# cyberfabric/cyberfabric-core

Measured on NVIDIA H100. Metric: prompt_bytes_per_sec_bpe_encode, higher is better.
Workload: dtype u32

## Files before the change

cyberfabric-core_b200/csrc/bpe_kernels.cuh:

```cuda
#pragma once
#include <stdint.h>

#include "pretok.cuh"
#include "pretok_fsm.h"
#include "pretok_sync.cuh"
#include "specials.h"
#include "tables.h"
#include "tma.cuh"

namespace cfbpe {

#ifdef CUSIM_EMULATOR
#define CFBPE_DYN_SMEM(name) uint32_t* const name = reinterpret_cast<uint32_t*>(cusim::dyn_smem())
#else
#define CFBPE_DYN_SMEM(name) extern __shared__ __align__(16) uint32_t name[]
#endif

constexpr uint32_t kMaxVocabs = 8;
#ifdef CUSIM_EMULATOR
inline unsigned long long* dbg_counters() { static unsigned long long c[16]; return c; }
#define CFBPE_DBG_COUNT(i) (++dbg_counters()[i])
#else
#define CFBPE_DBG_COUNT(i) ((void)0)
#endif
// ... 297 lines not shown
#endif
        }
    }
    if (!kFix) {
        or_bits(piece_bits, cs >> 5, static_cast<uint32_t>(mine));
        or_bits(piece_bits, (cs >> 5) + 1, static_cast<uint32_t>(mine >> 32));
    }
    if (bad) atomicOr(&status->bad_utf8, 1u);
}

__global__ void __launch_bounds__(256)
pretok_split_kernel(BatchView b, VocabSet vs, UcTables uc, uint32_t* __restrict__ piece_bits, DeviceStatus* status, SplitFix* fix_list, uint32_t fix_cap) {
    __shared__ uint16_t s_fsm[kNumPatterns * kPretokTableSize];
    __shared__ uint8_t s_ascii[128];
    for (uint32_t i = threadIdx.x; i < kNumPatterns * kPretokTableSize; i += blockDim.x) s_fsm[i] = uc.fsm[i];
    if (threadIdx.x < 128) s_ascii[threadIdx.x] = uc.ascii_x[threadIdx.x];
    __syncthreads();
    const uint64_t chunk = static_cast<uint64_t>(blockIdx.x) * blockDim.x + threadIdx.x;
    const uint64_t cs = chunk * kSplitChunk;
    if (cs >= b.total_bytes) return;
    const uint64_t ce = (cs + kSplitChunk < b.total_bytes) ? cs + kSplitChunk : b.total_bytes;
    split_thread<0>(b, vs, uc, s_fsm, s_ascii, piece_bits, status, fix_list, fix_cap, cs, ce, 0, 0);
}

__global__ void __launch_bounds__(256)
pretok_fixup_kernel(BatchView b, VocabSet vs, UcTables uc, uint32_t* __restrict__ piece_bits, DeviceStatus* status, const SplitFix* fix_list, uint32_t fix_cap) {
    __shared__ uint16_t s_fsm[kNumPatterns * kPretokTableSize];
    __shared__ uint8_t s_ascii[128];
    const uint32_t n = status->fix_n < fix_cap ? status->fix_n : fix_cap;
    if (blockIdx.x * blockDim.x >= n) return;
    for (uint32_t i = threadIdx.x; i < kNumPatterns * kPretokTableSize; i += blockDim.x) s_fsm[i] = uc.fsm[i];
    if (threadIdx.x < 128) s_ascii[threadIdx.x] = uc.ascii_x[threadIdx.x];
    __syncthreads();
    for (uint32_t i = blockIdx.x * blockDim.x + threadIdx.x; i < n; i += gridDim.x * blockDim.x) {
        const SplitFix f = fix_list[i];
        split_thread<1>(b, vs, uc, s_fsm, s_ascii, piece_bits, status, nullptr, 0, 0, f.ce, f.pos, 0xFFFFFFFFu);
    }
}


constexpr uint32_t kFull = 0xFFFFFFFFu;

__device__ __forceinline__ uint32_t lanemask_lt(uint32_t lane) { return (1u << lane) - 1u; }

__device__ __forceinline__ uint64_t load_bits33(const uint32_t* __restrict__ bits, uint64_t n_words, uint64_t ws) {
    const uint64_t w = ws >> 5;
    const uint32_t sh = static_cast<uint32_t>(ws & 31);
    const uint64_t lo = bits[w];
    const uint64_t hi = (w + 1 < n_words) ? bits[w + 1] : 0;
    const uint64_t v = (lo | (hi << 32)) >> sh;
    return v & 0x1FFFFFFFFull;
}

__device__ __forceinline__ uint64_t next_set_bit(const uint32_t* __restrict__ bits, uint64_t from, uint64_t limit) {
    if (from >= limit) return limit;
    uint64_t w = from >> 5;
    uint32_t cur = bits[w] & (kFull << (from & 31));
    const uint64_t wl = (limit + 31) >> 5;
    while (!cur) {
        if (++w >= wl) return limit;
        cur = bits[w];
    }
    const uint64_t p = (w << 5) + (__ffs(cur) - 1);
    return p < limit ? p : limit;
}


constexpr uint32_t kPieceRange = 512;
constexpr uint32_t kPieceWarps = 4;

__device__ __forceinline__ void load16(const uint8_t* __restrict__ p, uint32_t& w0, uint32_t& w1, uint32_t& w2, uint32_t& w3) {
    const uintptr_t addr = reinterpret_cast<uintptr_t>(p);
    const uint32_t* q = reinterpret_cast<const uint32_t*>(addr & ~static_cast<uintptr_t>(3));
    const uint32_t sh = static_cast<uint32_t>(addr & 3) * 8;
    const uint32_t a = q[0], bq = q[1], c = q[2], d = q[3];
    if (sh == 0) { w0 = a; w1 = bq; w2 = c; w3 = d; }
    else {
        const uint32_t e = q[4];
        w0 = __funnelshift_r(a, bq, sh); w1 = __funnelshift_r(bq, c, sh); w2 = __funnelshift_r(c, d, sh); w3 = __funnelshift_r(d, e, sh);
    }
}

__device__ __forceinline__ uint32_t whole_piece_lookup(const TablesView& T, const uint8_t* __restrict__ p, uint32_t len) {
    if (len > T.max_token_len) return kNone;
    uint32_t w0, w1, w2, w3;
    load16(p, w0, w1, w2, w3);
    uint64_t k0 = static_cast<uint64_t>(w0) | (static_cast<uint64_t>(w1) << 32);
    uint32_t k1 = w2;
    if (len < 8) k0 &= (1ull << (8 * len)) - 1ull;
    if (len <= 8) k1 = 0; else if (len < 12) k1 &= (1u << (8 * (len - 8))) - 1u;
    if (len <= kShortMaxLen) return short_lookup(T, k0, k1, len);
    return long_lookup(T, long_hash(k0, k1, load_le32(p + len - 4), len), p, len);
}

__device__ __forceinline__ uint32_t merge_piece_in_lane(const TablesView& T, const uint8_t* __restrict__ text, uint64_t pos, uint32_t len,
                                                        uint32_t* sid, uint32_t* srk, uint32_t* __restrict__ tok_bits) {
    const uint8_t* __restrict__ p = text + pos;
    uint32_t w[8];
    load16(p, w[0], w[1], w[2], w[3]);
    if (len > 16) load16(p + 16, w[4], w[5], w[6], w[7]); else { w[4] = w[5] = w[6] = w[7] = 0; }
    auto byte_at = [&](uint32_t k) -> uint32_t {
        const uint32_t lo4 = (k & 4u) ? ((k & 8u) ? ((k & 16u) ? w[7] : w[3]) : ((k & 16u) ? w[5] : w[1]))
                                       : ((k & 8u) ? ((k & 16u) ? w[6] : w[2]) : ((k & 16u) ? w[4] : w[0]));
        return (lo4 >> (8u * (k & 3u))) & 0xFFu;
    };
    for (uint32_t k0 = 0; k0 < len; k0 += 4) {
        uint32_t bv[5], idv[4], rkv[4];
#pragma unroll
        for (uint32_t t = 0; t < 5; ++t) bv[t] = (k0 + t < len) ? byte_at(k0 + t) : 0u;
#pragma unroll
        for (uint32_t t = 0; t < 4; ++t) {
            idv[t] = (k0 + t < len) ? T.byte2id[bv[t]] : 0u;
            rkv[t] = (k0 + t + 1 < len) ? T.bytepair[(bv[t] << 8) | bv[t + 1]] : kNone;
        }
#pragma unroll
        for (uint32_t t = 0; t < 4; ++t) if (k0 + t < len) { sid[(k0 + t) * 32] = idv[t]; srk[(k0 + t) * 32] = rkv[t] == kNone ? kNone : ((rkv[t] << 5) | (k0 + t)); }
    }
    uint32_t alive = (len >= 32) ? kFull : ((1u << len) - 1u);
    for (;;) {
        uint32_t bkey = kNone;
        for (uint32_t bits = alive; bits; bits &= bits - 1) {
            const uint32_t k = static_cast<uint32_t>(__ffs(bits)) - 1u;
            const uint32_t r = srk[k * 32];
            bkey = r < bkey ? r : bkey;
        }
        if (bkey == kNone) break;
        const uint32_t best = bkey >> 5, bi = bkey & 31u;
        const uint32_t above = alive & ~((2u << bi) - 1u);
        const uint32_t nb = static_cast<uint32_t>(__ffs(above)) - 1u;
        alive &= ~(1u << nb);
        sid[bi * 32] = best;
        const uint32_t above2 = alive & ~((2u << bi) - 1u);
        const uint32_t below = alive & ((1u << bi) - 1u);
        const bool wr = above2 != 0, wl = below != 0;
        const uint32_t nn = wr ? static_cast<uint32_t>(__ffs(above2)) - 1u : 0u;
        const uint32_t pv = wl ? 31u - static_cast<uint32_t>(__clz(below)) : 0u;
        uint32_t nr, nl;
        pair_lookup2(T, best, wr ? sid[nn * 32] : 0u, wr, wl ? sid[pv * 32] : 0u, best, wl, nr, nl);
        srk[bi * 32] = nr == kNone ? kNone : ((nr << 5) | bi);
        if (wl) srk[pv * 32] = nl == kNone ? kNone : ((nl << 5) | pv);
    }
    const uint64_t mask = static_cast<uint64_t>(alive) << (pos & 31);
    atomicOr(&tok_bits[pos >> 5], static_cast<uint32_t>(mask));
    if (mask >> 32) atomicOr(&tok_bits[(pos >> 5) + 1], static_cast<uint32_t>(mask >> 32));
    return alive;
}

__device__ __forceinline__ uint32_t kth_set_bit(uint32_t mask, uint32_t k) {
    for (uint32_t i = 0; i < k; ++i) mask &= mask - 1;
    return __ffs(mask) - 1;
}

constexpr uint32_t kPieceMulti = 0x80000000u;
constexpr uint32_t kPieceLong = 0xFFFFFFFEu;
constexpr uint32_t kPieceTileBytes = kPieceWarps * kPieceRange;
static_assert(kPieceTileBytes == 64 * 32, "K3 derives a word's piece tile as word >> 6");
struct DenseIds {
    uint32_t* by_piece;
    uint32_t* extras;
    uint32_t extras_cap;
    uint32_t* tile_pieces;
    uint64_t* piece_base;
};

__global__ void __launch_bounds__(kPieceWarps * 32)
long_scan_kernel(BatchView b, const uint32_t* __restrict__ piece_bits, LongPiece* __restrict__ long_list, uint32_t long_cap,
                 DeviceStatus* status, uint32_t* __restrict__ tile_pieces) {
    const uint32_t lane = threadIdx.x & 31, wic = threadIdx.x >> 5;
    const uint64_t warp = static_cast<uint64_t>(blockIdx.x) * kPieceWarps + wic;
    const uint64_t r0 = warp * kPieceRange;
    const uint64_t r1 = (r0 + kPieceRange < b.total_bytes) ? r0 + kPieceRange : b.total_bytes;
    const bool multi = b.vocab_ids != nullptr;
    const uint64_t base = r0 + 16ull * lane;
    const uint32_t my = (base < b.total_bytes) ? ((piece_bits[base >> 5] >> (16u * (lane & 1u))) & 0xFFFFu) : 0u;
    uint32_t v = my ? (16u * lane + static_cast<uint32_t>(__ffs(my)) - 1u) : 0xFFFFu;
#pragma unroll
    for (uint32_t d = 1; d < 32; d <<= 1) { const uint32_t o = __shfl_down_sync(kFull, v, d); if (lane + d < 32 && o < v) v = o; }
    uint32_t nf_rel = __shfl_down_sync(kFull, v, 1);
    if (lane == 31) nf_rel = 0xFFFFu;
    const bool any_open = __any_sync(kFull, my != 0 && nf_rel == 0xFFFFu);
    uint64_t beyond = b.total_bytes;
    if (any_open) beyond = next_set_bit(piece_bits, r1, b.total_bytes);
    const uint64_t nf = (nf_rel == 0xFFFFu) ? beyond : r0 + nf_rel;
    __shared__ uint32_t s_n[2], s_at[2], s_pieces;
    __shared__ unsigned long long s_bytes;
    if (threadIdx.x < 2) s_n[threadIdx.x] = 0;
    if (threadIdx.x == 0) { s_bytes = 0; s_pieces = 0; }
    __syncthreads();
    const uint32_t np = __reduce_add_sync(kFull, static_cast<uint32_t>(__popc(my)));
    if (lane == 0 && np) atomicAdd(&s_pieces, np);
    bool is_long = false, big = false;
    uint32_t k = 0, pv = 0;
    uint64_t pos = 0;
    if (my && r0 < b.total_bytes) {
        pos = base + (31u - static_cast<uint32_t>(__clz(my)));
        if (nf - pos > 32) {
            is_long = true;
            big = (nf - pos) > kBigPiece;
            pv = multi ? b.vocab_ids[find_prompt(b.offsets, b.n_prompts, pos)] : 0u;
            k = atomicAdd(&s_n[big ? 1 : 0], 1u);
            atomicAdd(&s_bytes, static_cast<unsigned long long>(nf - pos));
        }
    }
    __syncthreads();
    if (threadIdx.x < 2 && s_n[threadIdx.x]) s_at[threadIdx.x] = atomicAdd(threadIdx.x ? &status->n_big : &status->n_long, s_n[threadIdx.x]);
    if (threadIdx.x == 2 && s_bytes) atomicAdd(&status->long_bytes, s_bytes);
    if (threadIdx.x == 3) tile_pieces[blockIdx.x] = s_pieces;
    __syncthreads();
    if (is_long) {
        const uint32_t idx = s_at[big ? 1 : 0] + k;
        if (idx < long_cap) { LongPiece lp; lp.start = pos; lp.end = nf; lp.vocab = pv; lp.pad = 0; long_list[big ? long_cap - 1 - idx : idx] = lp; }
        else atomicOr(&status->long_overflow, 1u);
    }
}

constexpr uint32_t kLookupWarps = 4;
static_assert(kLookupWarps == kPieceWarps, "K2a's CTA is the 2 KiB tile K2s counted");
__global__ void __launch_bounds__(kLookupWarps * 32)
bpe_lookup_kernel(BatchView b, VocabSet vs, const uint32_t* __restrict__ piece_bits, DenseIds dn, MissLists ml, DeviceStatus* status) {
    __shared__ uint16_t s_pos[kLookupWarps][kPieceRange + 2];
    __shared__ uint64_t s_miss0[kLookupWarps * kPieceRange / 13 + 8];
    __shared__ uint64_t s_miss1[kLookupWarps * kPieceRange / 7 + 8];
    __shared__ uint64_t s_miss2[kLookupWarps * kPieceRange / 2 + 8];
    __shared__ uint32_t s_cnt[3], s_base[3], s_nw[kLookupWarps];
    const uint32_t lane = threadIdx.x & 31, wic = threadIdx.x >> 5;
    if (threadIdx.x < 3) s_cnt[threadIdx.x] = 0;
    const uint64_t warp = static_cast<uint64_t>(blockIdx.x) * kLookupWarps + wic;
    const uint64_t r0 = warp * kPieceRange;
    const uint8_t* __restrict__ text = b.bytes;
    const bool multi = b.vocab_ids != nullptr;
    const bool in_range = r0 < b.total_bytes;
    const uint64_t r1 = (r0 + kPieceRange < b.total_bytes) ? r0 + kPieceRange : b.total_bytes;
    uint32_t n_w = 0;
    if (in_range) {
        const uint64_t base = r0 + 16ull * lane;
// ... 1165 lines not shown
```

cyberfabric-core_b200/csrc/pipeline.cuh:

```cuda
#pragma once
#include "../../include/cfbpe.h"
#include "bpe_kernels.cuh"

namespace cfbpe {

struct Workspace {
    uint32_t* piece_bits;
    uint32_t* tok_bits;
    uint32_t* ids_by_pos;
    LongScratch lscratch;
    LongPiece* long_list;
    uint32_t long_cap;
    uint32_t* tile_counts;
    uint64_t* tile_base;
    DeviceStatus* status;
    MissLists miss;
    SplitFix* fix_list;
    uint32_t fix_cap;
    DenseIds dense;
    uint32_t* pstart_bits;
    uint32_t* block_prompt;
};

enum WsKind : uint32_t {
// ... 81 lines not shown
}

inline const char* chunk_args_error(uint32_t chunk_tokens, uint32_t overlap_tokens, const uint32_t* spans, const uint64_t* chunk_offsets) {
    if (chunk_tokens == 0) return "chunk_tokens must be at least 1";
    if (overlap_tokens >= chunk_tokens) return "overlap_tokens must be less than chunk_tokens";
    if (!spans || !chunk_offsets) return "out_spans and out_chunk_offsets are required";
    return nullptr;
}

#ifndef CFBPE_LONG_CTAS
#define CFBPE_LONG_CTAS 8
#endif
constexpr uint32_t kLongCtasPerSm = CFBPE_LONG_CTAS;
#ifndef CFBPE_LIST_CTAS
#define CFBPE_LIST_CTAS 3
#endif
constexpr uint32_t kListCtasPerSm = CFBPE_LIST_CTAS;

enum KernelIdx { K_SPLIT = 0, K_ENCODE = 1, K_LONG = 2, K_COUNT = 3, K_SCAN = 4, K_EMIT = 5, K_LIST = 6, K_LONGSCAN = 7, K_MERGE = 8 };

inline uint64_t n_flag_words(uint64_t total_bytes) { return (total_bytes + 31) >> 5; }
inline uint32_t n_scan_tiles(uint64_t total_bytes) {
    return static_cast<uint32_t>((n_flag_words(total_bytes) + kScanTileWords - 1) / kScanTileWords);
}

template <typename Stream, typename Prof>
inline void enqueue_split(const BatchView& b, const VocabSet& vs, const UcTables& uc, const Workspace& w, Stream stream, Prof* prof,
                          uint32_t sm_count) {
    const uint64_t nw = n_flag_words(b.total_bytes);
    CFBPE_ZERO(w.status, sizeof(DeviceStatus), stream);
    if (!b.total_bytes) return;
    CFBPE_ZERO(w.piece_bits, (nw + 2) * sizeof(uint32_t), stream);
    CFBPE_ZERO(w.tok_bits, (nw + 2) * sizeof(uint32_t), stream);
    CFBPE_MARK(prof, K_SPLIT, stream, true);
#ifdef CFBPE_SPLIT_LEGACY
    const uint64_t n_chunks = (b.total_bytes + kSplitChunk - 1) / kSplitChunk;
    CFBPE_LAUNCH(pretok_split_kernel, static_cast<unsigned>((n_chunks + 255) / 256), 256, stream, b, vs, uc, w.piece_bits, w.status, w.fix_list, w.fix_cap);
#else
    CFBPE_ZERO(w.pstart_bits, (nw + 2) * sizeof(uint32_t), stream);
    CFBPE_LAUNCH(prompt_map_kernel, static_cast<unsigned>((static_cast<uint64_t>(b.n_prompts) + 1 + 255) / 256), 256, stream, b, vs, w.pstart_bits, w.block_prompt, w.status);
    {
        const uint64_t n_blocks16 = (b.total_bytes + 15) / 16;
        const uint32_t n_tiles = static_cast<uint32_t>((n_blocks16 + kSplitWarpOwned - 1) / kSplitWarpOwned);
        const uint32_t n_tabs = b.vocab_ids ? kNumPatterns : 1u;
        const uint32_t cap = sm_count * CFBPE_SPLIT_CTAS;
        const uint32_t n_ctas = (n_tiles + kSplitCta / 32 - 1) / (kSplitCta / 32);
        CFBPE_LAUNCH_SMEM(pretok_split16_kernel, n_ctas < cap ? n_ctas : cap, kSplitCta, n_tabs * kProdTableBytes, stream,
                          b, vs, uc, w.pstart_bits, w.block_prompt, w.piece_bits, w.status, w.fix_list, w.fix_cap, n_tabs, n_tiles);
    }
#endif
    CFBPE_LAUNCH(pretok_fixup_kernel, 2 * sm_count, 256, stream, b, vs, uc, w.piece_bits, w.status, w.fix_list, w.fix_cap);
    CFBPE_MARK(prof, K_SPLIT, stream, false);
    const uint64_t n_warps = (b.total_bytes + kPieceRange - 1) / kPieceRange;
    CFBPE_MARK(prof, K_LONGSCAN, stream, true);
    CFBPE_LAUNCH(long_scan_kernel, static_cast<unsigned>((n_warps + kPieceWarps - 1) / kPieceWarps), kPieceWarps * 32, stream,
                 b, w.piece_bits, w.long_list, w.long_cap, w.status, w.dense.tile_pieces);
    CFBPE_MARK(prof, K_LONGSCAN, stream, false);
}

template <typename Stream, typename Prof>
inline void enqueue_short(const BatchView& b, const VocabSet& vs, const Workspace& w, uint32_t long_grid, Stream stream, Prof* prof) {
    if (!b.total_bytes) return;
    const uint64_t n_warps = (b.total_bytes + kPieceRange - 1) / kPieceRange;
    CFBPE_MARK(prof, K_ENCODE, stream, true);
    const uint32_t n_tiles2k = static_cast<uint32_t>((n_warps + kLookupWarps - 1) / kLookupWarps);
    CFBPE_LAUNCH(tile_scan_kernel, 1u, 1024, stream, w.dense.tile_pieces, n_tiles2k, w.dense.piece_base, static_cast<DeviceStatus*>(nullptr),
                 static_cast<const uint64_t*>(nullptr));
    CFBPE_LAUNCH(bpe_lookup_kernel, n_tiles2k, kLookupWarps * 32, stream, b, vs, w.piece_bits, w.dense, w.miss, w.status);
    CFBPE_MARK(prof, K_ENCODE, stream, false);
    CFBPE_MARK(prof, K_MERGE, stream, true);
    CFBPE_LAUNCH(bpe_merge_kernel, long_grid + long_grid / 2, kPieceWarps * 32, stream,
                 b, vs, w.piece_bits, w.dense, w.tok_bits, w.miss, w.status);
    CFBPE_MARK(prof, K_MERGE, stream, false);
}

template <typename Stream, typename Prof>
inline void enqueue_long(const BatchView& b, const VocabSet& vs, const Workspace& w, uint32_t long_grid, Stream stream, Prof* prof) {
    if (!b.total_bytes) return;
    CFBPE_MARK(prof, K_LONG, stream, true);
    CFBPE_LAUNCH(bpe_long_kernel, (long_grid / 4) * kLongCtasPerSm, kLongWarps * 32, stream, b, vs, w.long_list, w.status, w.long_cap, w.ids_by_pos, w.lscratch, w.tok_bits);
    CFBPE_MARK(prof, K_LONG, stream, false);
}
template <typename Stream, typename Prof>
inline void enqueue_list(const BatchView& b, const VocabSet& vs, const Workspace& w, uint32_t long_grid, Stream stream, Prof* prof) {
    if (!b.total_bytes) return;
#ifndef CFBPE_NO_DEFER
    CFBPE_MARK(prof, K_LIST, stream, true);
    CFBPE_LAUNCH_SMEM(bpe_list_kernel, (long_grid / 4) * kListCtasPerSm, kListWarps * 32, kListSmemBytes, stream, b, vs, w.long_list, w.status, w.long_cap, w.ids_by_pos, w.lscratch, w.tok_bits);
    CFBPE_MARK(prof, K_LIST, stream, false);
#endif
}

template <typename Stream, typename Prof>
inline void enqueue_count(const BatchView& b, const Workspace& w, Stream stream, Prof* prof) {
    if (!b.total_bytes) return;
    CFBPE_MARK(prof, K_COUNT, stream, true);
    CFBPE_LAUNCH(flag_count_kernel, n_scan_tiles(b.total_bytes), 256, stream, w.tok_bits, w.piece_bits, n_flag_words(b.total_bytes), w.tile_counts);
    CFBPE_MARK(prof, K_COUNT, stream, false);
}
template <typename Stream, typename Prof>
inline void enqueue_scan(const BatchView& b, const Workspace& w, Stream stream, Prof* prof, const uint64_t* token_base) {
    if (b.total_bytes) {
        CFBPE_MARK(prof, K_SCAN, stream, true);
        CFBPE_LAUNCH(tile_scan_kernel, 1u, 1024, stream, w.tile_counts, n_scan_tiles(b.total_bytes), w.tile_base, w.status, token_base);
        CFBPE_MARK(prof, K_SCAN, stream, false);
    } else {
        CFBPE_LAUNCH(tile_scan_kernel, 1u, 32, stream, w.tile_counts, 0u, w.tile_base, w.status, token_base);
    }
}
// ... 65 lines not shown
```

cyberfabric-core_b200/csrc/tables.h:

```cpp
#pragma once
#include <stdint.h>

#if defined(__CUDACC__)
#define CFBPE_HD __host__ __device__ __forceinline__
#else
#define CFBPE_HD inline
#endif

namespace cfbpe {

constexpr uint32_t kTablesMagic = 0x45504243u;
constexpr uint32_t kTablesVersion = 1;
constexpr uint32_t kNone = 0xFFFFFFFFu;
constexpr uint32_t kIdBits = 21;
constexpr uint32_t kIdMask = (1u << kIdBits) - 1;
constexpr uint64_t kPairEmpty = ~0ull;
constexpr uint32_t kShortMaxLen = 12;
constexpr uint32_t kMetaEmpty = 0xFFFFFFFFu;

struct TablesHeader {
    uint32_t magic, version;
    uint32_t n_ranks, pattern_id, max_token_len, n_pair_entries;
    uint64_t total_bytes;
    uint64_t off_byte2id;
    uint64_t off_bytepair;
    uint64_t off_pair;
    uint64_t off_short;
    uint64_t off_long;
    uint64_t off_tokoff;
    uint64_t off_blob;
    uint32_t cap_pair, cap_short, cap_long, blob_bytes;
    uint64_t content_hash;
};

struct ShortSlot { uint64_t k0; uint32_t k1; uint32_t meta; };
struct LongSlot { uint64_t hash; uint32_t meta; uint32_t blob_off; };

struct TablesView {
    const uint32_t* byte2id;
    const uint32_t* bytepair;
    const uint64_t* pair;
    const ShortSlot* shrt;
    const LongSlot* lng;
    const uint32_t* tokoff;
    const uint8_t* blob;
    uint32_t pair_mask, short_mask, long_mask;
    uint32_t n_ranks, pattern_id, max_token_len;
};

static inline TablesView make_view(const uint8_t* base, const TablesHeader& h) {
    TablesView v;
    v.byte2id = reinterpret_cast<const uint32_t*>(base + h.off_byte2id);
    v.bytepair = reinterpret_cast<const uint32_t*>(base + h.off_bytepair);
    v.pair = reinterpret_cast<const uint64_t*>(base + h.off_pair);
    v.shrt = reinterpret_cast<const ShortSlot*>(base + h.off_short);
    v.lng = reinterpret_cast<const LongSlot*>(base + h.off_long);
    v.tokoff = reinterpret_cast<const uint32_t*>(base + h.off_tokoff);
    v.blob = base + h.off_blob;
    v.pair_mask = h.cap_pair - 1;
    v.short_mask = h.cap_short - 1;
    v.long_mask = h.cap_long - 1;
    v.n_ranks = h.n_ranks;
    v.pattern_id = h.pattern_id;
    v.max_token_len = h.max_token_len;
    return v;
}

CFBPE_HD uint64_t mix64(uint64_t x) {
    x ^= x >> 30; x *= 0xbf58476d1ce4e5b9ull;
    x ^= x >> 27; x *= 0x94d049bb133111ebull;
    x ^= x >> 31;
    return x;
}
CFBPE_HD uint32_t mix32(uint32_t h) {
    h ^= h >> 16; h *= 0x21f0aaadu;
    h ^= h >> 15; h *= 0x735a2d97u;
    h ^= h >> 15;
    return h;
}
CFBPE_HD uint32_t pair_hash(uint32_t left, uint32_t right) {
    return mix32(left * 0x9E3779B1u + right * 0x85EBCA77u + 0x165667B1u);
}
CFBPE_HD uint64_t pair_slot(uint32_t left, uint32_t right, uint32_t merged) {
    return (static_cast<uint64_t>(left) << (2 * kIdBits)) | (static_cast<uint64_t>(right) << kIdBits) | merged;
}
CFBPE_HD uint32_t short_hash(uint64_t k0, uint32_t k1, uint32_t len) {
    const uint32_t lo = static_cast<uint32_t>(k0), hi = static_cast<uint32_t>(k0 >> 32);
    return mix32(lo * 0x9E3779B1u + hi * 0x85EBCA77u + k1 * 0xC2B2AE3Du + len * 0x27D4EB2Fu);
}
CFBPE_HD uint64_t long_hash(uint64_t k0, uint32_t k1, uint32_t last4, uint32_t len) {
    return mix64(k0 ^ mix64((static_cast<uint64_t>(k1) << 32) | last4) ^ (static_cast<uint64_t>(len) << 48));
}

CFBPE_HD uint32_t pair_lookup(const TablesView& t, uint32_t left, uint32_t right) {
    const uint64_t key = (static_cast<uint64_t>(left) << kIdBits) | right;
    uint32_t h = pair_hash(left, right) & t.pair_mask;
    for (;;) {
        const uint64_t s = t.pair[h];
        if ((s >> kIdBits) == key) return static_cast<uint32_t>(s) & kIdMask;
        if (s == kPairEmpty) return kNone;
        h = (h + 1) & t.pair_mask;
    }
}
CFBPE_HD void pair_lookup2(const TablesView& t, uint32_t l0, uint32_t r0, bool want0, uint32_t l1, uint32_t r1, bool want1,
                           uint32_t& out0, uint32_t& out1) {
    const uint64_t key0 = (static_cast<uint64_t>(l0) << kIdBits) | r0, key1 = (static_cast<uint64_t>(l1) << kIdBits) | r1;
    uint32_t h0 = pair_hash(l0, r0) & t.pair_mask, h1 = pair_hash(l1, r1) & t.pair_mask;
    uint64_t s0 = want0 ? t.pair[h0] : kPairEmpty;
    uint64_t s1 = want1 ? t.pair[h1] : kPairEmpty;
    out0 = kNone; out1 = kNone;
    for (;;) {
// ... 70 lines not shown
```

cyberfabric-core_b200/csrc/vocab.cpp:

```cpp
#include "vocab.h"

#include <cstring>
#include <string_view>
#include <unordered_map>

#include "../../include/cfbpe.h"

namespace cfbpe {

namespace {

int b64val(int c) {
    if (c >= 'A' && c <= 'Z') return c - 'A';
    if (c >= 'a' && c <= 'z') return c - 'a' + 26;
    if (c >= '0' && c <= '9') return c - '0' + 52;
    if (c == '+') return 62;
    if (c == '/') return 63;
    return -1;
}

bool b64decode(const uint8_t* p, size_t n, std::string& out) {
    out.clear();
    uint32_t acc = 0;
    int bits = 0;
// ... 100 lines not shown
        if (i < len && f[i] == ']') break;
        if (i < len && f[i] == ',') { ++i; continue; }
        if (i >= len || f[i] != '{') { err = "tekken json: expected object in vocab"; return CFBPE_EINVAL; }
        ++i;
        bool have_rank = false, have_bytes = false;
        uint64_t rank = 0;
        for (;;) {
            skip_ws();
            if (i < len && f[i] == '}') { ++i; break; }
            if (i < len && f[i] == ',') { ++i; continue; }
            size_t ks, ke;
            if (!read_string(ks, ke)) { err = "tekken json: expected key"; return CFBPE_EINVAL; }
            std::string_view k(reinterpret_cast<const char*>(f) + ks, ke - ks);
            skip_ws();
            if (i >= len || f[i] != ':') { err = "tekken json: expected ':'"; return CFBPE_EINVAL; }
            ++i; skip_ws();
            if (i < len && f[i] == '"') {
                size_t vs, ve;
                if (!read_string(vs, ve)) { err = "tekken json: bad string"; return CFBPE_EINVAL; }
                if (k == "token_bytes") {
                    if (!b64decode(f + vs, ve - vs, tb) || tb.empty()) { err = "tekken json: bad base64"; return CFBPE_EINVAL; }
                    have_bytes = true;
                }
            } else {
                size_t vs = i;
                while (i < len && f[i] != ',' && f[i] != '}' && f[i] != ' ' && f[i] != '\n') ++i;
                if (k == "rank") {
                    rank = 0;
                    for (size_t j = vs; j < i; ++j) {
                        if (f[j] < '0' || f[j] > '9') { err = "tekken json: bad rank"; return CFBPE_EINVAL; }
                        rank = rank * 10 + (f[j] - '0');
                        if (rank > kMaxRank) { err = "tekken json: rank too large"; return CFBPE_EINVAL; }
                    }
                    have_rank = true;
                }
            }
        }
        if (!have_rank || !have_bytes) { err = "tekken json: vocab entry without rank/token_bytes"; return CFBPE_EINVAL; }
        if (!max_ranks || rank < max_ranks) {
            if (rank < seen.size() && seen[rank]) { err = "tekken json: duplicate rank"; return CFBPE_EINVAL; }
            put_token(tokens, seen, rank, std::move(tb));
        }
    }
    return finish_tokens(tokens, seen, max_ranks, err);
}

namespace {
uint32_t pow2_at_least(uint64_t x) {
    uint32_t c = 16;
    while (c < x) c <<= 1;
    return c;
}
uint64_t align_up(uint64_t x, uint64_t a) { return (x + a - 1) / a * a; }
}

int build_tables(const std::vector<std::string>& tokens, uint32_t pattern_id, std::vector<uint8_t>& blob,
                 std::string& err) {
    const uint32_t n = static_cast<uint32_t>(tokens.size());
    if (n < 256 || n > kMaxRank) { err = "vocab size out of range"; return CFBPE_EINVAL; }
    if (pattern_id >= CFBPE_PATTERN_COUNT) { err = "unknown pattern id"; return CFBPE_EINVAL; }

    std::unordered_map<std::string_view, uint32_t> index;
    index.reserve(n * 2);
    uint32_t max_len = 0;
    uint64_t blob_bytes = 0;
    for (uint32_t r = 0; r < n; ++r) {
        const std::string& t = tokens[r];
        if (t.empty()) { err = "empty token at rank " + std::to_string(r); return CFBPE_EINVAL; }
        if (t.size() > 255) { err = "token longer than 255 bytes at rank " + std::to_string(r); return CFBPE_EINVAL; }
        if (!index.emplace(std::string_view(t), r).second) { err = "duplicate token bytes at rank " + std::to_string(r); return CFBPE_EINVAL; }
        if (t.size() > max_len) max_len = static_cast<uint32_t>(t.size());
        blob_bytes += t.size();
    }
    uint32_t byte2id[256];
    for (int b = 0; b < 256; ++b) {
        char c = static_cast<char>(b);
        auto it = index.find(std::string_view(&c, 1));
        if (it == index.end()) { err = "byte " + std::to_string(b) + " is not in the vocabulary"; return CFBPE_EINVAL; }
        byte2id[b] = it->second;
    }

    struct PairE { uint32_t l, r, m; };
    std::vector<PairE> pairs;
    pairs.reserve(static_cast<size_t>(n) * 5 / 2);
    uint32_t n_short = 0, n_long = 0;
    for (uint32_t id = 0; id < n; ++id) {
        const std::string& t = tokens[id];
        if (t.size() <= kShortMaxLen) ++n_short; else ++n_long;
        std::string_view sv(t);
        for (size_t k = 1; k < t.size(); ++k) {
            auto il = index.find(sv.substr(0, k));
            if (il == index.end()) continue;
            auto ir = index.find(sv.substr(k));
            if (ir == index.end()) continue;
            pairs.push_back({il->second, ir->second, id});
        }
    }

    TablesHeader h{};
    h.magic = kTablesMagic;
    h.version = kTablesVersion;
    h.n_ranks = n;
    h.pattern_id = pattern_id;
    h.max_token_len = max_len;
    h.n_pair_entries = static_cast<uint32_t>(pairs.size());
    h.cap_pair = pow2_at_least(pairs.size() * 4 + 16);
    h.cap_short = pow2_at_least(static_cast<uint64_t>(n_short) * 2 + 16);
    h.cap_long = pow2_at_least(static_cast<uint64_t>(n_long) * 2 + 16);
    h.blob_bytes = static_cast<uint32_t>(blob_bytes);
    uint64_t off = align_up(sizeof(TablesHeader), 256);
    h.off_byte2id = off;  off = align_up(off + 256 * 4, 256);
    h.off_bytepair = off; off = align_up(off + 65536 * 4, 256);
    h.off_pair = off;     off = align_up(off + static_cast<uint64_t>(h.cap_pair) * 8, 256);
    h.off_short = off;    off = align_up(off + static_cast<uint64_t>(h.cap_short) * sizeof(ShortSlot), 256);
    h.off_long = off;     off = align_up(off + static_cast<uint64_t>(h.cap_long) * sizeof(LongSlot), 256);
    h.off_tokoff = off;   off = align_up(off + (static_cast<uint64_t>(n) + 1) * 4, 256);
    h.off_blob = off;     off = align_up(off + blob_bytes + 16, 256);
    h.total_bytes = off;

    blob.assign(off, 0);
    uint8_t* base = blob.data();
    std::memcpy(base + h.off_byte2id, byte2id, sizeof byte2id);

    uint32_t* bytepair = reinterpret_cast<uint32_t*>(base + h.off_bytepair);
    for (uint32_t i = 0; i < 65536; ++i) bytepair[i] = kNone;
    uint64_t* pt = reinterpret_cast<uint64_t*>(base + h.off_pair);
    for (uint32_t i = 0; i < h.cap_pair; ++i) pt[i] = kPairEmpty;
    for (const PairE& p : pairs) {
        uint32_t s = pair_hash(p.l, p.r) & (h.cap_pair - 1);
        while (pt[s] != kPairEmpty) s = (s + 1) & (h.cap_pair - 1);
        pt[s] = pair_slot(p.l, p.r, p.m);
    }
    for (uint32_t id = 0; id < n; ++id) {
        const std::string& t = tokens[id];
        if (t.size() == 2) bytepair[(static_cast<uint8_t>(t[0]) << 8) | static_cast<uint8_t>(t[1])] = id;
    }

    ShortSlot* st = reinterpret_cast<ShortSlot*>(base + h.off_short);
    for (uint32_t i = 0; i < h.cap_short; ++i) st[i] = ShortSlot{0, 0, kMetaEmpty};
    LongSlot* lt = reinterpret_cast<LongSlot*>(base + h.off_long);
    for (uint32_t i = 0; i < h.cap_long; ++i) lt[i] = LongSlot{0, kMetaEmpty, 0};
    uint32_t* tokoff = reinterpret_cast<uint32_t*>(base + h.off_tokoff);
    uint8_t* bytes = base + h.off_blob;
    uint32_t bo = 0;
    uint64_t ch = 1469598103934665603ull;
    for (uint32_t id = 0; id < n; ++id) {
        const std::string& t = tokens[id];
        const uint32_t len = static_cast<uint32_t>(t.size());
        tokoff[id] = bo;
        std::memcpy(bytes + bo, t.data(), len);
        const uint8_t* p = bytes + bo;
        ch = (ch ^ len) * 1099511628211ull;
        for (uint32_t i = 0; i < len; ++i) ch = (ch ^ p[i]) * 1099511628211ull;
        uint64_t k0; uint32_t k1;
        pack_key(p, len, k0, k1);
        if (len <= kShortMaxLen) {
            uint32_t s = short_hash(k0, k1, len) & (h.cap_short - 1);
            while (st[s].meta != kMetaEmpty) s = (s + 1) & (h.cap_short - 1);
            st[s] = ShortSlot{k0, k1, (len << 24) | id};
        } else {
            const uint64_t hv = long_hash(k0, k1, load_le32(p + len - 4), len);
            uint32_t s = static_cast<uint32_t>(hv >> 17) & (h.cap_long - 1);
            while (lt[s].meta != kMetaEmpty) s = (s + 1) & (h.cap_long - 1);
            lt[s] = LongSlot{hv, (len << 24) | id, bo};
        }
        bo += len;
    }
    tokoff[n] = bo;
    h.content_hash = ch;
    std::memcpy(base, &h, sizeof h);
    return CFBPE_OK;
}

int validate_tables(const uint8_t* blob, uint64_t size, std::string& err) {
    if (size < sizeof(TablesHeader)) { err = "table blob too small"; return CFBPE_EINVAL; }
    TablesHeader h;
    std::memcpy(&h, blob, sizeof h);
    auto pow2 = [](uint32_t x) { return x && !(x & (x - 1)); };
    if (h.magic != kTablesMagic || h.version != kTablesVersion) { err = "table blob: bad magic/version"; return CFBPE_EINVAL; }
    if (h.total_bytes != size) { err = "table blob: size mismatch"; return CFBPE_EINVAL; }
    if (!pow2(h.cap_pair) || !pow2(h.cap_short) || !pow2(h.cap_long)) { err = "table blob: capacities"; return CFBPE_EINVAL; }
    if (h.n_ranks < 256 || h.n_ranks > kMaxRank || h.pattern_id >= CFBPE_PATTERN_COUNT || h.max_token_len > 255) { err = "table blob: header fields"; return CFBPE_EINVAL; }
    auto inside = [&](uint64_t off, uint64_t bytes) { return off % 16 == 0 && off <= size && bytes <= size - off; };
    if (!inside(h.off_byte2id, 1024) || !inside(h.off_bytepair, 65536 * 4) ||
        !inside(h.off_pair, static_cast<uint64_t>(h.cap_pair) * 8) ||
        !inside(h.off_short, static_cast<uint64_t>(h.cap_short) * sizeof(ShortSlot)) ||
        !inside(h.off_long, static_cast<uint64_t>(h.cap_long) * sizeof(LongSlot)) ||
        !inside(h.off_tokoff, (static_cast<uint64_t>(h.n_ranks) + 1) * 4) ||
        !inside(h.off_blob, static_cast<uint64_t>(h.blob_bytes) + 16)) { err = "table blob: section out of bounds"; return CFBPE_EINVAL; }
    const uint64_t* pairs = reinterpret_cast<const uint64_t*>(blob + h.off_pair);
    uint64_t free_pairs = 0;
    for (uint32_t i = 0; i < h.cap_pair; ++i) {
        const uint64_t sl = pairs[i];
        if (sl == kPairEmpty) { ++free_pairs; continue; }
        const uint32_t l = static_cast<uint32_t>(sl >> (2 * kIdBits)), r = static_cast<uint32_t>(sl >> kIdBits) & kIdMask, m = static_cast<uint32_t>(sl) & kIdMask;
        if (l >= h.n_ranks || r >= h.n_ranks || m >= h.n_ranks) { err = "table blob: pair entry names an id outside the vocabulary"; return CFBPE_EINVAL; }
    }
    if (free_pairs * 2 < h.cap_pair) { err = "table blob: pair table more than half full"; return CFBPE_EINVAL; }
    const ShortSlot* st = reinterpret_cast<const ShortSlot*>(blob + h.off_short);
    uint64_t free_short = 0;
    for (uint32_t i = 0; i < h.cap_short; ++i) {
        if (st[i].meta == kMetaEmpty) { ++free_short; continue; }
        if ((st[i].meta & 0x00FFFFFFu) >= h.n_ranks || (st[i].meta >> 24) > kShortMaxLen) { err = "table blob: short-token entry out of range"; return CFBPE_EINVAL; }
    }
    const LongSlot* lt = reinterpret_cast<const LongSlot*>(blob + h.off_long);
    uint64_t free_long = 0;
    for (uint32_t i = 0; i < h.cap_long; ++i) {
        if (lt[i].meta == kMetaEmpty) { ++free_long; continue; }
        const uint32_t len = lt[i].meta >> 24;
        if ((lt[i].meta & 0x00FFFFFFu) >= h.n_ranks || static_cast<uint64_t>(lt[i].blob_off) + len > h.blob_bytes) { err = "table blob: long-token entry out of range"; return CFBPE_EINVAL; }
    }
    if (!free_short || !free_long) { err = "table blob: a token table has no free slot"; return CFBPE_EINVAL; }
    const uint32_t* tokoff = reinterpret_cast<const uint32_t*>(blob + h.off_tokoff);
    const uint32_t* byte2id = reinterpret_cast<const uint32_t*>(blob + h.off_byte2id);
    const uint32_t* bytepair = reinterpret_cast<const uint32_t*>(blob + h.off_bytepair);
    for (uint32_t i = 0; i < h.n_ranks; ++i)
        if (tokoff[i] > tokoff[i + 1] || tokoff[i + 1] - tokoff[i] > 255) { err = "table blob: token offsets"; return CFBPE_EINVAL; }
    if (tokoff[0] != 0 || tokoff[h.n_ranks] != h.blob_bytes) { err = "table blob: token offsets do not cover the byte blob"; return CFBPE_EINVAL; }
    for (uint32_t i = 0; i < 256; ++i) if (byte2id[i] != kNone && byte2id[i] >= h.n_ranks) { err = "table blob: byte table"; return CFBPE_EINVAL; }
    for (uint32_t i = 0; i < 65536; ++i) if (bytepair[i] != kNone && bytepair[i] >= h.n_ranks) { err = "table blob: byte-pair table"; return CFBPE_EINVAL; }
    const uint8_t* bytes = blob + h.off_blob;
    uint64_t ch = 1469598103934665603ull;
    for (uint32_t id = 0; id < h.n_ranks; ++id) {
        const uint32_t len = tokoff[id + 1] - tokoff[id];
        ch = (ch ^ len) * 1099511628211ull;
        for (uint32_t i = 0; i < len; ++i) ch = (ch ^ bytes[tokoff[id] + i]) * 1099511628211ull;
    }
    if (ch != h.content_hash) { err = "table blob: content hash mismatch"; return CFBPE_EINVAL; }
    return CFBPE_OK;
}

}
```

Measured before the change: 36.04 billion.

## Split long pieces at provably independent byte boundaries using bigram/trigram cut tables

Adds vocabulary-derived bigram and trigram tables, built on the host when tables are created, that prove when a byte boundary can never be merged across by BPE. A new piece_cut_kernel scans each 16-byte group, finds positions inside long pre-token pieces where no merge can span, and marks them as extra piece starts. long_scan then merges these cuts into piece_bits, so long pieces are broken into shorter independent pieces that take the cheaper short-piece path. In exchange it adds an extra kernel pass with random lookups into a 2 MB trigram bitmap, grows the table format, and relies on a subtle correctness argument about when cuts are safe.

```diff
diff --git a/cyberfabric-core_b200/csrc/bpe_kernels.cuh b/cyberfabric-core_b200/csrc/bpe_kernels.cuh
--- a/cyberfabric-core_b200/csrc/bpe_kernels.cuh
+++ b/cyberfabric-core_b200/csrc/bpe_kernels.cuh
@@ -373,14 +373,15 @@
     return v & 0x1FFFFFFFFull;
 }
 
-__device__ __forceinline__ uint64_t next_set_bit(const uint32_t* __restrict__ bits, uint64_t from, uint64_t limit) {
+__device__ __forceinline__ uint64_t next_set_bit(const uint32_t* __restrict__ bits, uint64_t from, uint64_t limit,
+                                                 const uint32_t* __restrict__ also = nullptr) {
     if (from >= limit) return limit;
     uint64_t w = from >> 5;
-    uint32_t cur = bits[w] & (kFull << (from & 31));
+    uint32_t cur = (bits[w] | (also ? also[w] : 0u)) & (kFull << (from & 31));
     const uint64_t wl = (limit + 31) >> 5;
     while (!cur) {
         if (++w >= wl) return limit;
-        cur = bits[w];
+        cur = bits[w] | (also ? also[w] : 0u);
     }
     const uint64_t p = (w << 5) + (__ffs(cur) - 1);
     return p < limit ? p : limit;
@@ -484,16 +485,109 @@
     uint64_t* piece_base;
 };
 
+__device__ __forceinline__ bool bit_set(const uint32_t* __restrict__ bits, uint32_t i) { return (bits[i >> 5] >> (i & 31u)) & 1u; }
+
+__device__ __forceinline__ uint32_t piece_cuts16(const BatchView& b, const VocabSet& vs, const uint32_t* __restrict__ piece_bits, uint64_t base) {
+    const uint64_t W = base >> 5;
+    const uint32_t h = static_cast<uint32_t>(base & 16u);
+    unsigned __int128 s = (static_cast<unsigned __int128>(piece_bits[W + 1]) << 64) | (static_cast<unsigned __int128>(piece_bits[W]) << 32) |
+                          (W ? piece_bits[W - 1] : kFull);
+    const uint64_t from_end = b.total_bytes + 32 - 32 * W;
+    if (from_end < 96) s |= ~static_cast<unsigned __int128>(0) << from_end;
+    unsigned __int128 r = ~s & ((static_cast<unsigned __int128>(1) << 96) - 1);
+    r &= r >> 1; r &= r >> 2; r &= r >> 4; r &= r >> 8; r &= r >> 16;
+    unsigned __int128 c = r;
+    c |= c << 1; c |= c << 2; c |= c << 4; c |= c << 8; c |= c << 16;
+    uint32_t todo = static_cast<uint32_t>(c >> (32 + h)) & 0xFFFFu;
+    if (!todo) return 0;
+    const uint32_t starts = static_cast<uint32_t>(s >> (24 + h));
+    uint32_t pre, wv[7];
+    load16(b.bytes + base, wv[1], wv[2], wv[3], wv[4]);
+    pre = base ? load_u32_any(b.bytes + base - 8) : 0u;
+    wv[0] = base ? load_u32_any(b.bytes + base - 4) : 0u;
+    wv[5] = load_u32_any(b.bytes + base + 16);
+    wv[6] = load_u32_any(b.bytes + base + 20);
+    auto byte_at = [&](uint32_t i) -> uint32_t { return (wv[i >> 2] >> (8u * (i & 3u))) & 0xFFu; };
+    auto three_at = [&](int i) -> uint32_t {
+        uint32_t v = 0;
+        for (int t = 0; t < 3; ++t) v |= (i + t < 0 ? (pre >> (8 * (i + t + 4))) & 0xFFu : byte_at(static_cast<uint32_t>(i + t))) << (8 * t);
+        return v;
+    };
+#pragma unroll
+    for (uint32_t k = 0; k < 16; ++k) {
+        if (!((todo >> k) & 1u)) continue;
+        const uint32_t left = three_at(static_cast<int>(k) + 1), right = three_at(static_cast<int>(k) + 4);
+#pragma unroll
+        for (uint32_t q = 1; q <= 5; ++q) {
+            const bool in_left = !((starts >> (k + 6 - q)) & ((4u << q) - 1u)) && three_at(static_cast<int>(k + 1 - q)) == left;
+            const bool in_right = !((starts >> (k + 9)) & ((4u << q) - 1u)) && three_at(static_cast<int>(k + 4 + q)) == right;
+            if (in_left || in_right) { todo &= ~(1u << k); break; }
+        }
+    }
+    uint32_t cuts = 0;
+    while (todo) {
+        uint32_t mine = todo;
+        TablesView T = vs.v[0];
+        if (b.vocab_ids) {
+            const uint32_t p = find_prompt(b.offsets, b.n_prompts, base + static_cast<uint32_t>(__ffs(todo)) - 1u);
+            T = vs.v[b.vocab_ids[p]];
+            const uint64_t pe = b.offsets[p + 1];
+            if (pe < base + 16) mine &= (1u << (pe - base)) - 1u;
+        }
+        todo &= ~mine;
+        if (!T.cut2) continue;
+        uint32_t need = 0;
+#pragma unroll
+        for (uint32_t k = 0; k < 16; ++k) {
+            if (!((mine >> k) & 1u)) continue;
+            if (!bit_set(T.cut2, (byte_at(k + 3) << 8) | byte_at(k + 4))) cuts |= 1u << k;
+            else need |= 1u << k;
+        }
+#pragma unroll 1
+        for (uint32_t g = 0; g < 2; ++g) {
+            if (!((need >> (8 * g)) & 0xFFu)) continue;
+            const uint32_t w0 = g ? wv[2] : wv[0], w1 = g ? wv[3] : wv[1], w2 = g ? wv[4] : wv[2], w3 = g ? wv[5] : wv[3];
+            auto gbyte = [&](uint32_t i) -> uint32_t {
+                return ((i < 4 ? w0 : i < 8 ? w1 : i < 12 ? w2 : w3) >> (8u * (i & 3u))) & 0xFFu;
+            };
+#pragma unroll
+            for (uint32_t t = 0; t < 8; ++t) {
+                const uint32_t k = 8 * g + t;
+                if (!((need >> k) & 1u)) continue;
+                const uint32_t x = gbyte(t + 3), y = gbyte(t + 4);
+                const bool pair_is_token = T.bytepair[(x << 8) | y] != kNone;
+                const bool t1 = !((starts >> (k + 7)) & 1u) && bit_set(T.cut3, (gbyte(t + 2) << 16) | (x << 8) | y);
+                const bool t2 = !((starts >> (k + 9)) & 1u) && bit_set(T.cut3, (x << 16) | (y << 8) | gbyte(t + 5));
+                if (!pair_is_token && !t1 && !t2) cuts |= 1u << k;
+            }
+        }
+    }
+    return cuts;
+}
+
 __global__ void __launch_bounds__(kPieceWarps * 32)
-long_scan_kernel(BatchView b, const uint32_t* __restrict__ piece_bits, LongPiece* __restrict__ long_list, uint32_t long_cap,
-                 DeviceStatus* status, uint32_t* __restrict__ tile_pieces) {
+piece_cut_kernel(BatchView b, VocabSet vs, const uint32_t* __restrict__ piece_bits, uint32_t* __restrict__ cut_bits) {
+    const uint64_t base = (static_cast<uint64_t>(blockIdx.x) * kPieceWarps + (threadIdx.x >> 5)) * kPieceRange + 16ull * (threadIdx.x & 31u);
+    const uint32_t cuts = base < b.total_bytes ? piece_cuts16(b, vs, piece_bits, base) << (base & 16u) : 0u;
+    const uint32_t word = cuts | __shfl_xor_sync(kFull, cuts, 1);
+    if (!(base & 16u) && word) cut_bits[base >> 5] = word;
+}
+
+__global__ void __launch_bounds__(kPieceWarps * 32)
+long_scan_kernel(BatchView b, uint32_t* __restrict__ piece_bits, const uint32_t* __restrict__ cut_bits, LongPiece* __restrict__ long_list,
+                 uint32_t long_cap, DeviceStatus* status, uint32_t* __restrict__ tile_pieces) {
     const uint32_t lane = threadIdx.x & 31, wic = threadIdx.x >> 5;
     const uint64_t warp = static_cast<uint64_t>(blockIdx.x) * kPieceWarps + wic;
     const uint64_t r0 = warp * kPieceRange;
     const uint64_t r1 = (r0 + kPieceRange < b.total_bytes) ? r0 + kPieceRange : b.total_bytes;
     const bool multi = b.vocab_ids != nullptr;
     const uint64_t base = r0 + 16ull * lane;
-    const uint32_t my = (base < b.total_bytes) ? ((piece_bits[base >> 5] >> (16u * (lane & 1u))) & 0xFFFFu) : 0u;
+    uint32_t my = 0;
+    if (base < b.total_bytes) {
+        const uint32_t cw = cut_bits[base >> 5], pw = piece_bits[base >> 5];
+        if (cw && !(lane & 1u)) piece_bits[base >> 5] = pw | cw;
+        my = ((pw | cw) >> (16u * (lane & 1u))) & 0xFFFFu;
+    }
     uint32_t v = my ? (16u * lane + static_cast<uint32_t>(__ffs(my)) - 1u) : 0xFFFFu;
 #pragma unroll
     for (uint32_t d = 1; d < 32; d <<= 1) { const uint32_t o = __shfl_down_sync(kFull, v, d); if (lane + d < 32 && o < v) v = o; }
@@ -501,7 +595,7 @@
     if (lane == 31) nf_rel = 0xFFFFu;
     const bool any_open = __any_sync(kFull, my != 0 && nf_rel == 0xFFFFu);
     uint64_t beyond = b.total_bytes;
-    if (any_open) beyond = next_set_bit(piece_bits, r1, b.total_bytes);
+    if (any_open) beyond = next_set_bit(piece_bits, r1, b.total_bytes, cut_bits);
     const uint64_t nf = (nf_rel == 0xFFFFu) ? beyond : r0 + nf_rel;
     __shared__ uint32_t s_n[2], s_at[2], s_pieces;
     __shared__ unsigned long long s_bytes;
diff --git a/cyberfabric-core_b200/csrc/pipeline.cuh b/cyberfabric-core_b200/csrc/pipeline.cuh
--- a/cyberfabric-core_b200/csrc/pipeline.cuh
+++ b/cyberfabric-core_b200/csrc/pipeline.cuh
@@ -157,9 +157,11 @@
     CFBPE_LAUNCH(pretok_fixup_kernel, 2 * sm_count, 256, stream, b, vs, uc, w.piece_bits, w.status, w.fix_list, w.fix_cap);
     CFBPE_MARK(prof, K_SPLIT, stream, false);
     const uint64_t n_warps = (b.total_bytes + kPieceRange - 1) / kPieceRange;
+    const unsigned n_ctas = static_cast<unsigned>((n_warps + kPieceWarps - 1) / kPieceWarps);
     CFBPE_MARK(prof, K_LONGSCAN, stream, true);
-    CFBPE_LAUNCH(long_scan_kernel, static_cast<unsigned>((n_warps + kPieceWarps - 1) / kPieceWarps), kPieceWarps * 32, stream,
-                 b, w.piece_bits, w.long_list, w.long_cap, w.status, w.dense.tile_pieces);
+    CFBPE_LAUNCH(piece_cut_kernel, n_ctas, kPieceWarps * 32, stream, b, vs, w.piece_bits, w.tok_bits);
+    CFBPE_LAUNCH(long_scan_kernel, n_ctas, kPieceWarps * 32, stream, b, w.piece_bits, w.tok_bits, w.long_list, w.long_cap, w.status,
+                 w.dense.tile_pieces);
     CFBPE_MARK(prof, K_LONGSCAN, stream, false);
 }
 
diff --git a/cyberfabric-core_b200/csrc/tables.h b/cyberfabric-core_b200/csrc/tables.h
--- a/cyberfabric-core_b200/csrc/tables.h
+++ b/cyberfabric-core_b200/csrc/tables.h
@@ -10,7 +10,7 @@
 namespace cfbpe {
 
 constexpr uint32_t kTablesMagic = 0x45504243u;
-constexpr uint32_t kTablesVersion = 1;
+constexpr uint32_t kTablesVersion = 2;
 constexpr uint32_t kNone = 0xFFFFFFFFu;
 constexpr uint32_t kIdBits = 21;
 constexpr uint32_t kIdMask = (1u << kIdBits) - 1;
@@ -31,7 +31,13 @@
     uint64_t off_blob;
     uint32_t cap_pair, cap_short, cap_long, blob_bytes;
     uint64_t content_hash;
+    uint64_t off_cut2;
+    uint64_t off_cut3;
+    uint32_t cuts_ok;
+    uint32_t pad0;
 };
+constexpr uint32_t kCut2Words = 65536 / 32;
+constexpr uint32_t kCut3Words = (1u << 24) / 32;
 
 struct ShortSlot { uint64_t k0; uint32_t k1; uint32_t meta; };
 struct LongSlot { uint64_t hash; uint32_t meta; uint32_t blob_off; };
@@ -44,6 +50,8 @@
     const LongSlot* lng;
     const uint32_t* tokoff;
     const uint8_t* blob;
+    const uint32_t* cut2;
+    const uint32_t* cut3;
     uint32_t pair_mask, short_mask, long_mask;
     uint32_t n_ranks, pattern_id, max_token_len;
 };
@@ -57,6 +65,8 @@
     v.lng = reinterpret_cast<const LongSlot*>(base + h.off_long);
     v.tokoff = reinterpret_cast<const uint32_t*>(base + h.off_tokoff);
     v.blob = base + h.off_blob;
+    v.cut2 = h.cuts_ok ? reinterpret_cast<const uint32_t*>(base + h.off_cut2) : nullptr;
+    v.cut3 = reinterpret_cast<const uint32_t*>(base + h.off_cut3);
     v.pair_mask = h.cap_pair - 1;
     v.short_mask = h.cap_short - 1;
     v.long_mask = h.cap_long - 1;
diff --git a/cyberfabric-core_b200/csrc/vocab.cpp b/cyberfabric-core_b200/csrc/vocab.cpp
--- a/cyberfabric-core_b200/csrc/vocab.cpp
+++ b/cyberfabric-core_b200/csrc/vocab.cpp
@@ -176,6 +176,45 @@
     return c;
 }
 uint64_t align_up(uint64_t x, uint64_t a) { return (x + a - 1) / a * a; }
+
+bool build_cut_tables(const std::vector<std::string_view>& tokens, uint32_t* cut2, uint32_t* cut3) {
+    std::unordered_map<std::string_view, uint32_t> index;
+    index.reserve(tokens.size() * 2);
+    for (uint32_t r = 0; r < tokens.size(); ++r) index.emplace(tokens[r], r);
+    bool reachable = true;
+    std::vector<uint32_t> start, rank;
+    for (const std::string_view t : tokens) {
+        const size_t n = t.size();
+        for (size_t i = 0; i + 1 < n; ++i) {
+            const uint32_t a = static_cast<uint8_t>(t[i]), b = static_cast<uint8_t>(t[i + 1]);
+            cut2[((a << 8) | b) >> 5] |= 1u << (b & 31);
+            if (i + 2 < n) {
+                const uint32_t g = (a << 16) | (b << 8) | static_cast<uint8_t>(t[i + 2]);
+                cut3[g >> 5] |= 1u << (g & 31);
+            }
+        }
+        if (n < 2 || !reachable) continue;
+        auto pair_rank = [&](size_t k) {
+            const auto it = index.find(t.substr(start[k], start[k + 2] - start[k]));
+            return it == index.end() ? kNone : it->second;
+        };
+        start.resize(n + 1);
+        for (size_t i = 0; i <= n; ++i) start[i] = static_cast<uint32_t>(i);
+        rank.assign(n - 1, kNone);
+        for (size_t k = 0; k + 1 < n; ++k) rank[k] = pair_rank(k);
+        while (!rank.empty()) {
+            size_t best = 0;
+            for (size_t k = 1; k < rank.size(); ++k) if (rank[k] < rank[best]) best = k;
+            if (rank[best] == kNone) break;
+            start.erase(start.begin() + static_cast<std::ptrdiff_t>(best) + 1);
+            rank.erase(rank.begin() + static_cast<std::ptrdiff_t>(best));
+            if (best < rank.size()) rank[best] = pair_rank(best);
+            if (best > 0) rank[best - 1] = pair_rank(best - 1);
+        }
+        reachable = rank.empty();
+    }
+    return reachable;
+}
 }
 
 int build_tables(const std::vector<std::string>& tokens, uint32_t pattern_id, std::vector<uint8_t>& blob,
@@ -240,6 +279,8 @@
     h.off_long = off;     off = align_up(off + static_cast<uint64_t>(h.cap_long) * sizeof(LongSlot), 256);
     h.off_tokoff = off;   off = align_up(off + (static_cast<uint64_t>(n) + 1) * 4, 256);
     h.off_blob = off;     off = align_up(off + blob_bytes + 16, 256);
+    h.off_cut2 = off;     off = align_up(off + kCut2Words * 4, 256);
+    h.off_cut3 = off;     off = align_up(off + static_cast<uint64_t>(kCut3Words) * 4, 256);
     h.total_bytes = off;
 
     blob.assign(off, 0);
@@ -292,6 +333,8 @@
     }
     tokoff[n] = bo;
     h.content_hash = ch;
+    h.cuts_ok = build_cut_tables(std::vector<std::string_view>(tokens.begin(), tokens.end()), reinterpret_cast<uint32_t*>(base + h.off_cut2),
+                                 reinterpret_cast<uint32_t*>(base + h.off_cut3)) ? 1u : 0u;
     std::memcpy(base, &h, sizeof h);
     return CFBPE_OK;
 }
@@ -311,7 +354,8 @@
         !inside(h.off_short, static_cast<uint64_t>(h.cap_short) * sizeof(ShortSlot)) ||
         !inside(h.off_long, static_cast<uint64_t>(h.cap_long) * sizeof(LongSlot)) ||
         !inside(h.off_tokoff, (static_cast<uint64_t>(h.n_ranks) + 1) * 4) ||
-        !inside(h.off_blob, static_cast<uint64_t>(h.blob_bytes) + 16)) { err = "table blob: section out of bounds"; return CFBPE_EINVAL; }
+        !inside(h.off_blob, static_cast<uint64_t>(h.blob_bytes) + 16) || !inside(h.off_cut2, kCut2Words * 4) ||
+        !inside(h.off_cut3, static_cast<uint64_t>(kCut3Words) * 4)) { err = "table blob: section out of bounds"; return CFBPE_EINVAL; }
     const uint64_t* pairs = reinterpret_cast<const uint64_t*>(blob + h.off_pair);
     uint64_t free_pairs = 0;
     for (uint32_t i = 0; i < h.cap_pair; ++i) {
@@ -351,6 +395,12 @@
         for (uint32_t i = 0; i < len; ++i) ch = (ch ^ bytes[tokoff[id] + i]) * 1099511628211ull;
     }
     if (ch != h.content_hash) { err = "table blob: content hash mismatch"; return CFBPE_EINVAL; }
+    std::vector<std::string_view> toks(h.n_ranks);
+    for (uint32_t id = 0; id < h.n_ranks; ++id) toks[id] = std::string_view(reinterpret_cast<const char*>(bytes) + tokoff[id], tokoff[id + 1] - tokoff[id]);
+    std::vector<uint32_t> cut2(kCut2Words, 0), cut3(kCut3Words, 0);
+    const uint32_t cuts_ok = build_cut_tables(toks, cut2.data(), cut3.data()) ? 1u : 0u;
+    if (cuts_ok != h.cuts_ok || std::memcmp(cut2.data(), blob + h.off_cut2, kCut2Words * 4) ||
+        std::memcmp(cut3.data(), blob + h.off_cut3, static_cast<size_t>(kCut3Words) * 4)) { err = "table blob: cut tables do not match the tokens"; return CFBPE_EINVAL; }
     return CFBPE_OK;
 }
 
```

Measured after the change: 36.99 billion (median of 6 runs). 2.6% higher.
